# XinMing0411/zero-shot-AAC

Hardware: AMD Instinct MI355X
Metric: audio clips/sec end-to-end (encode+mapper+GPT-2 decode), Clotho-eval bs=64 (higher is better)
Workload: dtype bf16

## Files before the change

### zero-shot-aac_amd/csrc/decode_grid.hip

```cpp
#include <type_traits>

#include "common.h"

#pragma clang fp contract(off)

namespace zs {
int g_dp_spin = 0;
int g_dg_exp = 0;
int g_dg_dynf = 1;
int g_dp_abort = -1;
int g_dg_win_lo = 0;
int g_dg_win_hi = 62;
namespace dg {

constexpr int D = 768, NH = 12, HD = 64, DFF = 3072, NLY = 12, RM = 64, QKVN = 3 * D;
constexpr int NW = 4, NT = 64 * NW;
constexpr int KSD = D / 32, KSF = DFF / 32;
constexpr int QS = KSD / NW, QF = KSF / NW;
constexpr int NCB_Q = QKVN / 16, NCB_D = D / 16, NCB_F = DFF / 16;
constexpr unsigned SPIN_MAX = 1u << 22;
#ifndef DG_NSH
#define DG_NSH 8
#endif
constexpr int NSH = DG_NSH;
// ... 262 lines not shown
typedef __attribute__((ext_vector_type(2))) float f32x2_t;
__device__ __forceinline__ float dot2bf(unsigned x, unsigned y, float c) {
  return __builtin_amdgcn_fdot2_f32_bf16(__builtin_bit_cast(bf16x2_t, x), __builtin_bit_cast(bf16x2_t, y),
                                         c, false);
}
template <int NRB>
__device__ __forceinline__ void ln_stats(const u32x4_t* xf, const Sm& sm, int rb0) {
  const int tid = otid(), v = tid >> 6, lane = tid & 63, fr = lane & 15;
  constexpr unsigned ONE2 = 0x3f803f80u;
#pragma unroll
  for (int rb = 0; rb < NRB; ++rb) {
    float s = 0.f, q = 0.f;
#pragma unroll
    for (int i = 0; i < QS; ++i) {
      const u32x4_t u = xf[rb * QS + i];
      s = dot2bf(u.x, ONE2, s); q = dot2bf(u.x, u.x, q);
      s = dot2bf(u.y, ONE2, s); q = dot2bf(u.y, u.y, q);
      s = dot2bf(u.z, ONE2, s); q = dot2bf(u.z, u.z, q);
      s = dot2bf(u.w, ONE2, s); q = dot2bf(u.w, u.w, q);
    }
    s = add32(add16(s));
    q = add32(add16(q));
    if (lane < 16) {
      sm.ln[v * RM + 16 * (rb0 + rb) + fr] = s;
      sm.ln[(NW + v) * RM + 16 * (rb0 + rb) + fr] = q;
    }
  }
}
__device__ __forceinline__ void ln_row(const Sm& sm, int r, float& mean, float& rstd) {
  const float* l2 = sm.ln + NW * RM;
  mean = ((sm.ln[r] + sm.ln[RM + r]) + (sm.ln[2 * RM + r] + sm.ln[3 * RM + r])) * (1.0f / D);
  const float ex2 = ((l2[r] + l2[RM + r]) + (l2[2 * RM + r] + l2[3 * RM + r])) * (1.0f / D);
  rstd = rsqrtf(fmaxf(fmaf(-mean, mean, ex2), 0.f) + 1e-5f);
}
template <int NC>
__device__ __forceinline__ void stage_cb(const Sm& sm, const float* b2, int N, int n0) {
  static_assert(NC <= 64, "SM_CB holds 64 columns");
  const int t = otid();
  if (t < NC) sm.cb[t] = b2[n0 + t];
  else if (t >= 64 && t < 64 + NC) sm.cb[t] = b2[N + n0 + t - 64];
}
__device__ __forceinline__ float4 cb_quad(const Sm& sm, int lc, int row1) {
  return *reinterpret_cast<const float4*>(sm.cb + 64 * row1 + lc);
}
__device__ __forceinline__ float4 ln_fold(f32x4_t s, float mean, float rstd, float4 cs, float4 b) {
  return make_float4(fmaf(rstd, fmaf(-mean, cs.x, s[0]), b.x), fmaf(rstd, fmaf(-mean, cs.y, s[1]), b.y),
                     fmaf(rstd, fmaf(-mean, cs.z, s[2]), b.z), fmaf(rstd, fmaf(-mean, cs.w, s[3]), b.w));
}

template <int NRB>
__device__ __forceinline__ void embed_frags(const Args& a, const Sm& sm, int rb0, u32x4_t* xf) {
  const int tid = otid(), v = tid >> 6, lane = tid & 63, fr = lane & 15, fk = 8 * (lane >> 4);
#pragma unroll
  for (int rb = 0; rb < NRB; ++rb) {
    const int row = 16 * (rb0 + rb) + fr;
    const bf16_t* te = a.wte + (long)sm.tok[row] * D + fk;
#pragma unroll
    for (int i = 0; i < QS; ++i)
      xf[rb * QS + i] = *reinterpret_cast<const u32x4_t*>(te + 32 * (QS * v + i));
  }
#pragma unroll
  for (int rb = 0; rb < NRB; ++rb) {
    const int row = 16 * (rb0 + rb) + fr;
    const bf16_t* pe = a.wpe + (long)sm.pos[row] * D + fk;
    u32x4_t pu[QS];
#pragma unroll
    for (int i = 0; i < QS; ++i) pu[i] = *reinterpret_cast<const u32x4_t*>(pe + 32 * (QS * v + i));
#pragma unroll
    for (int i = 0; i < QS; ++i) {
      float t[8], p[8];
      unpack8(xf[rb * QS + i], t);
      unpack8(pu[i], p);
#pragma unroll
      for (int e = 0; e < 8; ++e) t[e] += p[e];
      xf[rb * QS + i] = pack8(t);
    }
  }
}
__device__ __forceinline__ float4 embed_quad(const Args& a, const Sm& sm, int row, int col) {
  const uint2 t = *reinterpret_cast<const uint2*>(a.wte + (long)sm.tok[row] * D + col);
  const uint2 p = *reinterpret_cast<const uint2*>(a.wpe + (long)sm.pos[row] * D + col);
  return make_float4(__uint_as_float(t.x << 16) + __uint_as_float(p.x << 16),
                     __uint_as_float(t.x & 0xffff0000u) + __uint_as_float(p.x & 0xffff0000u),
                     __uint_as_float(t.y << 16) + __uint_as_float(p.y << 16),
                     __uint_as_float(t.y & 0xffff0000u) + __uint_as_float(p.y & 0xffff0000u));
}

template <int CB, int RB>
struct Rounds {
  static constexpr int CPR = CB < 8 / RB ? CB : 8 / RB;
  static constexpr int NR = (CB + CPR - 1) / CPR;
  static constexpr int NJ = (CPR * RB + NW - 1) / NW;
};
template <int CB, int RB, int PF, typename LoadW, typename Epi>
__device__ __forceinline__ void gemm_rounds(const u32x4_t* xf, u32x4_t* wpf, f32x4_t* red,
                                            LoadW&& loadw, Epi&& epi) {
  constexpr int CPR = Rounds<CB, RB>::CPR, NR = Rounds<CB, RB>::NR;
  static_assert(PF == CB || PF == CPR, "weight prefetch rounds");
  static_for<NR>([&](auto rr) {
    constexpr int r = decltype(rr)::value, c0 = r * CPR;
    constexpr int NC = CB - c0 < CPR ? CB - c0 : CPR;
    f32x4_t acc[NC * RB];
#pragma unroll
    for (int t = 0; t < NC * RB; ++t) acc[t] = f32x4_t{0.f, 0.f, 0.f, 0.f};
#pragma unroll
    for (int s = 0; s < QS; ++s)
#pragma unroll
      for (int c = 0; c < NC; ++c)
#pragma unroll
        for (int rb = 0; rb < RB; ++rb)
          acc[c * RB + rb] = mfma(wpf[((PF == CB ? c0 : 0) + c) * QS + s], xf[rb * QS + s], acc[c * RB + rb]);
    if constexpr (PF != CB && c0 + CPR < CB) {
      loadw(c0 + CPR, std::integral_constant<int, (CB - c0 - CPR < CPR ? CB - c0 - CPR : CPR)>{}, wpf);
      __builtin_amdgcn_sched_barrier(0);
    }
    reduce_tiles<NC * RB>(red, acc, [&](int j, int t, f32x4_t s) { epi(r, j, c0 + t / RB, t % RB, s); });
  });
}

template <int G, bool PM>
__device__ __forceinline__ void phase_a(const Args& a, const Rs& rs, int l, int w, const Sm& sm,
                                        u32x4_t* wq) {
  using Gm = Geo<G>;
  constexpr int CB = Gm::ACB, RB = Gm::ARB, NCG = NCB_Q / CB;
  const int tid = otid(), v = tid >> 6, lane = tid & 63;
  const int cb0 = (w % NCG) * CB, rb0 = (w / NCG) * RB;
  u32x4_t xf[RB * QS];
  if (l == 0) embed_frags<RB>(a, sm, rb0, xf);
  else lda<RB, QS>(rs.xb, KSD, rb0, QS * v, xf);
  if constexpr (PM) ldw<Gm::APF, QS>(a.wq[l], KSD, cb0, QS * v, wq);
  stage_cb<16 * CB>(sm, a.bq[l], QKVN, 16 * cb0);
  __builtin_amdgcn_sched_barrier(0);
  ln_stats<RB>(xf, sm, rb0);
  const __amdgpu_buffer_rsrc_t rk = mk(a.kc[l], a.kv_bytes), rv = mk(a.vc[l], a.kv_bytes);
  gemm_rounds<CB, RB, Gm::APF>(xf, wq, sm.red,
      [&](int c, auto n, u32x4_t* wr) { ldw<decltype(n)::value, QS>(a.wq[l], KSD, cb0 + c, QS * (otid() >> 6), wr); },
      [&](int r, int j, int c, int rb, f32x4_t s) {
        const int row = 16 * (rb0 + rb) + (lane & 15), col = 16 * (cb0 + c) + 4 * (lane >> 4);
        if (row >= a.R) return;
        float mean, rstd;
        ln_row(sm, row, mean, rstd);
        const int lc = 16 * c + 4 * (lane >> 4);
        const float4 o4 = ln_fold(s, mean, rstd, cb_quad(sm, lc, 1), cb_quad(sm, lc, 0));
        const u32x2_t o{pk2bf(o4.x, o4.y), pk2bf(o4.z, o4.w)};
        if (col < D) {
          st8(rs.q, (row * D + col) * 2, o);
        } else {
          const int j = col - D, kv = j >= D, jj = kv ? j - D : j;
          const int off = ((((row * NH + jj / HD) * a.Lmax) + sm.pos[row]) * HD + (jj % HD)) * 2;
          st8(kv ? rv : rk, off, o);
        }
      });
}

__device__ __forceinline__ float gelu_new_fast(float x) {
  const float u2 = -1.5957691216057308f * fmaf(0.044715f * x * x, x, x);
  return x * __builtin_amdgcn_rcpf(1.0f + __expf(u2));
}
template <int G, bool PM>
__device__ __forceinline__ void phase_d(const Args& a, const Rs& rs, int l, int w, const Sm& sm,
                                        u32x4_t* wf) {
  using Gm = Geo<G>;
  constexpr int CB = Gm::DCB, RB = Gm::DRB, NCG = NCB_F / CB;
  const int tid = otid(), v = tid >> 6, lane = tid & 63;
  const int cb0 = (w % NCG) * CB, rb0 = (w / NCG) * RB;
  u32x4_t xf[RB * QS];
  lda<RB, QS>(rs.xb, KSD, rb0, QS * v, xf);
  if constexpr (PM) ldw<Gm::DPF, QS>(a.wf[l], KSD, cb0, QS * v, wf);
  stage_cb<16 * CB>(sm, a.bfc[l], DFF, 16 * cb0);
  __builtin_amdgcn_sched_barrier(0);
  ln_stats<RB>(xf, sm, rb0);
  gemm_rounds<CB, RB, Gm::DPF>(xf, wf, sm.red,
      [&](int c, auto n, u32x4_t* wr) { ldw<decltype(n)::value, QS>(a.wf[l], KSD, cb0 + c, QS * (otid() >> 6), wr); },
      [&](int r, int j, int c, int rb, f32x4_t s) {
        const int row = 16 * (rb0 + rb) + (lane & 15), col = 16 * (cb0 + c) + 4 * (lane >> 4);
        if (row >= a.R) return;
        float mean, rstd;
        ln_row(sm, row, mean, rstd);
        const int lc = 16 * c + 4 * (lane >> 4);
        const float4 h = ln_fold(s, mean, rstd, cb_quad(sm, lc, 1), cb_quad(sm, lc, 0));
        st8(rs.hid, frag_off(row, col, KSF),
            u32x2_t{pk2bf(gelu_new_fast(h.x), gelu_new_fast(h.y)),
                    pk2bf(gelu_new_fast(h.z), gelu_new_fast(h.w))});
      });
}

template <int G>
__device__ __forceinline__ void ce_tile(int w, int t, int& row, int& col) {
  using Gm = Geo<G>;
  constexpr int NCG = NCB_D / Gm::ECB;
  const int lane = otid() & 63;
  const int cb0 = (w % NCG) * Gm::ECB, rb0 = (w / NCG) * Gm::ERB;
  row = 16 * (rb0 + t % Gm::ERB) + (lane & 15);
  col = 16 * (cb0 + t / Gm::ERB) + 4 * (lane >> 4);
}
template <int G, bool PM>
__device__ __forceinline__ void ce_operands(const Args& a, const Sm& sm, bool embed, int w,
                                            const float* bias, const f32x4_t& xo, float4& b,
                                            float4& xold) {
  constexpr int T = Geo<G>::ECB * Geo<G>::ERB;
  const int v = otid() >> 6;
  b = make_float4(0.f, 0.f, 0.f, 0.f);
  xold = b;
  if (v < T) {
    int row, col;
    ce_tile<G>(w, v, row, col);
    b = *reinterpret_cast<const float4*>(bias + col);
    if (embed) {
      xold = embed_quad(a, sm, row, col);
    } else if constexpr (PM) {
      xold = *reinterpret_cast<const float4*>(reinterpret_cast<const float*>(a.ws + WS_X) + row * D + col);
    } else {
      xold = make_float4(xo[0], xo[1], xo[2], xo[3]);
    }
  }
}
template <int G, bool PM>
__device__ __forceinline__ void ce_epilogue(const Args& a, const Rs& rs, int w, int t, f32x4_t s,
                                            const float4& b, const float4& xold, f32x4_t& xo) {
  int row, col;
  ce_tile<G>(w, t, row, col);
  const f32x4_t o{(s[0] + b.x) + xold.x, (s[1] + b.y) + xold.y, (s[2] + b.z) + xold.z,
                  (s[3] + b.w) + xold.w};
  xo = o;
  if (row < a.R) {
    st8(rs.xb, frag_off(row, col, KSD), u32x2_t{pk2bf(o[0], o[1]), pk2bf(o[2], o[3])});
    if constexpr (PM)
      *reinterpret_cast<float4*>(reinterpret_cast<float*>(a.ws + WS_X) + row * D + col) =
          make_float4(o[0], o[1], o[2], o[3]);
  }
}

template <int G, bool PM>
__device__ __forceinline__ void phase_c(const Args& a, const Rs& rs, int l, int w, const Sm& sm,
                                        u32x4_t* wo, f32x4_t& xo) {
  using Gm = Geo<G>;
  constexpr int CB = Gm::ECB, RB = Gm::ERB, T = CB * RB, NCG = NCB_D / CB;
  const int v = otid() >> 6;
  const int cb0 = (w % NCG) * CB, rb0 = (w / NCG) * RB;
  u32x4_t af[RB * QS];
  lda<RB, QS>(rs.att, KSD, rb0, QS * v, af);
  if constexpr (PM) ldw<CB, QS>(a.wo[l], KSD, cb0, QS * v, wo);
  float4 b, xold;
  ce_operands<G, PM>(a, sm, l == 0, w, a.bo[l], xo, b, xold);
  __builtin_amdgcn_sched_barrier(0);
  f32x4_t acc[T];
#pragma unroll
  for (int t = 0; t < T; ++t) acc[t] = f32x4_t{0.f, 0.f, 0.f, 0.f};
#pragma unroll
  for (int s = 0; s < QS; ++s)
#pragma unroll
    for (int c = 0; c < CB; ++c)
#pragma unroll
      for (int rb = 0; rb < RB; ++rb) acc[c * RB + rb] = mfma(wo[c * QS + s], af[rb * QS + s], acc[c * RB + rb]);
  reduce_tiles<T>(sm.red, acc, [&](int, int t, f32x4_t s) { ce_epilogue<G, PM>(a, rs, w, t, s, b, xold, xo); });
}

template <int G, bool PM>
__device__ __forceinline__ void phase_e(const Args& a, const Rs& rs, int l, int w, const Sm& sm,
                                        u32x4_t* wm, f32x4_t& xo) {
  using Gm = Geo<G>;
  constexpr int CB = Gm::ECB, RB = Gm::ERB, T = CB * RB, NCG = NCB_D / CB, NCH = QF / ECH, ESL = Gm::ESL;
  const int v = otid() >> 6;
  const int cb0 = (w % NCG) * CB, rb0 = (w / NCG) * RB, s0 = QF * v;
  if constexpr (PM) {
#pragma unroll
    for (int k = 0; k < ESL; ++k) ldw<CB, ECH>(a.wm[l], KSF, cb0, s0 + ECH * k, wm + k * CB * ECH);
  }
  u32x4_t af[ESL * RB * ECH];
#pragma unroll
  for (int k = 0; k < ESL; ++k) lda<RB, ECH>(rs.hid, KSF, rb0, s0 + ECH * k, af + k * RB * ECH);
  float4 b, xold;
  ce_operands<G, PM>(a, sm, false, w, a.bm[l], xo, b, xold);
  __builtin_amdgcn_sched_barrier(0);
  f32x4_t acc[T];
#pragma unroll
  for (int t = 0; t < T; ++t) acc[t] = f32x4_t{0.f, 0.f, 0.f, 0.f};
  static_for<NCH>([&](auto cc) {
    constexpr int c = decltype(cc)::value, sl = c % ESL;
#pragma unroll
    for (int s = 0; s < ECH; ++s)
#pragma unroll
      for (int cb = 0; cb < CB; ++cb)
#pragma unroll
        for (int rb = 0; rb < RB; ++rb)
          acc[cb * RB + rb] = mfma(wm[(sl * CB + cb) * ECH + s], af[(sl * RB + rb) * ECH + s], acc[cb * RB + rb]);
    if constexpr (c + ESL < NCH) {
      ldw<CB, ECH>(a.wm[l], KSF, cb0, s0 + ECH * (c + ESL), wm + sl * CB * ECH);
      lda<RB, ECH>(rs.hid, KSF, rb0, s0 + ECH * (c + ESL), af + sl * RB * ECH);
      __builtin_amdgcn_sched_barrier(0);
    }
  });
  reduce_tiles<T>(sm.red, acc, [&](int, int t, f32x4_t s) { ce_epilogue<G, PM>(a, rs, w, t, s, b, xold, xo); });
}

__device__ __forceinline__ void attn_unit(const Args& a, const Sm& sm, int u, int& row, int& hh,
                                          int& p, long& base) {
  row = u / NH;
  hh = u % NH;
  const int rr = min(row, a.R - 1);
  p = (a.exp & 2) ? 1 : min(sm.pos[rr], a.Lmax - 1);
  base = ((long)(rr * NH + hh) * a.Lmax) * HD + 8 * ((otid() & 63) & 7);
}
template <int KU, int KC>
__device__ __forceinline__ void attn_load(const Args& a, int l, const Sm& sm, int ub, int cb,
                                          u32x4_t (&kr)[KU][KC], u32x4_t (&vr)[KU][KC]) {
  const int tid = otid(), v = tid >> 6, grp = (tid & 63) >> 3;
  const bf16_t* kc = a.kc[l];
  const bf16_t* vc = a.vc[l];
#pragma unroll
  for (int k = 0; k < KU; ++k) {
    int row, hh, p;
    long base;
    attn_unit(a, sm, ub + KU * v + k, row, hh, p, base);
#pragma unroll
    for (int i = 0; i < KC; ++i) {
      const int jc = max(min(cb + 8 * i + grp, p - 1), 0);
      kr[k][i] = __builtin_nontemporal_load(reinterpret_cast<const u32x4_t*>(kc + base + (long)jc * HD));
      vr[k][i] = __builtin_nontemporal_load(reinterpret_cast<const u32x4_t*>(vc + base + (long)jc * HD));
    }
  }
}
template <int KU, int KC>
__device__ __forceinline__ void phase_b(const Args& a, const Rs& rs, int l, const Sm& sm, int ub,
                                        u32x4_t (&kr)[KU][KC], u32x4_t (&vr)[KU][KC]) {
  const int tid = otid(), lane = tid & 63, v = tid >> 6, grp = lane >> 3, sub = lane & 7;
  const __amdgpu_buffer_rsrc_t rk = mk(a.kc[l], a.kv_bytes), rv = mk(a.vc[l], a.kv_bytes);
  float m[KU], sum[KU];
  f32x2_t o[KU][4];
  int p[KU], row[KU], hh[KU];
  long base[KU];
  u32x4_t qu[KU], knu[KU], vnu[KU];
#pragma unroll
  for (int k = 0; k < KU; ++k) {
    attn_unit(a, sm, ub + KU * v + k, row[k], hh[k], p[k], base[k]);
    qu[k] = ld16(rs.q, (min(row[k], a.R - 1) * D + hh[k] * HD + 8 * sub) * 2);
    const int off = (int)((base[k] + (long)p[k] * HD) * 2);
    knu[k] = ld16(rk, off);
    vnu[k] = ld16(rv, off);
  }
  __builtin_amdgcn_sched_barrier(0);
  auto qk = [&](const u32x4_t& qv, const u32x4_t& kv) {
    float sv = dot2bf(qv.x, kv.x, 0.f);
    sv = dot2bf(qv.y, kv.y, sv);
    sv = dot2bf(qv.z, kv.z, sv);
    sv = dot2bf(qv.w, kv.w, sv);
    return sum8(sv) * 0.125f;
  };
#pragma unroll
  for (int k = 0; k < KU; ++k) {
    m[k] = qk(qu[k], knu[k]);
    sum[k] = grp == 0 ? 1.f : 0.f;
    const unsigned w[4] = {vnu[k].x, vnu[k].y, vnu[k].z, vnu[k].w};
#pragma unroll
    for (int t = 0; t < 4; ++t)
      o[k][t] = grp == 0 ? f32x2_t{__uint_as_float(w[t] << 16), __uint_as_float(w[t] & 0xffff0000u)}
                         : f32x2_t{0.f, 0.f};
  }
  auto vacc = [&](f32x2_t (&acc)[4], float e, const u32x4_t& vv) {
    const unsigned w[4] = {vv.x, vv.y, vv.z, vv.w};
    const f32x2_t e2 = {e, e};
#pragma unroll
    for (int t = 0; t < 4; ++t)
      acc[t] = __builtin_elementwise_fma(e2, f32x2_t{__uint_as_float(w[t] << 16),
                                                     __uint_as_float(w[t] & 0xffff0000u)}, acc[t]);
  };
  int pmax = p[0];
#pragma unroll
  for (int k = 1; k < KU; ++k) pmax = max(pmax, p[k]);
  for (int cb = 0; cb < pmax; cb += 8 * KC) {
    if (cb > 0) attn_load<KU, KC>(a, l, sm, ub, cb, kr, vr);
#pragma unroll
    for (int h = 0; h < KC / 4; ++h) {
      const int cs = cb + 32 * h;
#pragma unroll
      for (int k = 0; k < KU; ++k) {
        if (cs >= p[k]) continue;
        float sc[4];
        float pm = -INFINITY;
#pragma unroll
        for (int i = 0; i < 4; ++i) {
          const float sv = qk(qu[k], kr[k][4 * h + i]);
          sc[i] = cs + 8 * i + grp < p[k] ? sv : -INFINITY;
          pm = fmaxf(pm, sc[i]);
        }
        pm = fmaxf(pm, xor8(pm));
        pm = max16(pm);
        pm = max32(pm);
        const float mn = fmaxf(m[k], pm);
        const float scale = __expf(m[k] - mn);
        sum[k] *= scale;
        const f32x2_t sc2 = {scale, scale};
#pragma unroll
        for (int t = 0; t < 4; ++t) o[k][t] *= sc2;
        m[k] = mn;
#pragma unroll
        for (int i = 0; i < 4; ++i) {
          const float e = __expf(sc[i] - mn);
          sum[k] += e;
          vacc(o[k], e, vr[k][4 * h + i]);
        }
      }
    }
  }
#pragma unroll
  for (int k = 0; k < KU; ++k) {
    const float inv = 1.0f / add32(add16(sum[k] + xor8(sum[k])));
    float of[8];
#pragma unroll
    for (int t = 0; t < 4; ++t) {
      of[2 * t] = add32(add16(o[k][t].x + xor8(o[k][t].x))) * inv;
      of[2 * t + 1] = add32(add16(o[k][t].y + xor8(o[k][t].y))) * inv;
    }
    if (grp == 0 && row[k] < a.R) {
      const int r = row[k];
      st16(rs.att, (((r >> 4) * KSD + 2 * hh[k] + (sub >> 2)) * 64 + (r & 15) + 16 * (sub & 3)) * 16,
           pack8(of));
    }
  }
}

template <int G, bool DYN>
__device__ __forceinline__ void phase_f(const Args& a, const Rs& rs, int w, const Sm& sm, gu64* keys,
                                        gu32* fctr) {
  const int tid = otid(), v = tid >> 6, lane = tid & 63;
  u32x4_t xf[4 * QS];
  lda<4, QS>(rs.xb, KSD, 0, QS * v, xf);
  const int nvb = (a.V + 15) >> 4, lmv = 16 * nvb;
  constexpr int NSL = Geo<G>::FSL;
  int su = (nvb + G * NSL - 1) / (G * NSL);
  bool dyn = false;
  if constexpr (DYN) {
    const int s2 = max(3, (nvb * 5 / 8) / (G * NSL));
    if (G * NSL * s2 <= nvb - G && a.exp == 0 && a.dynf) { su = s2; dyn = true; }
  }
  const int d0 = G * NSL * su, nch = dyn ? (nvb - d0 + NSL - 1) / NSL : 0;
  int* const chr = sm.misc + 12;
  auto iter_blocks = [&](int u, int& b0, int& st) {
    if (u < su) { b0 = w + G * NSL * u; st = G; }
    else if (dyn) { b0 = d0 + NSL * __builtin_amdgcn_readfirstlane(chr[u & 3]); st = 1; }
    else { b0 = 0x3fffffff; st = 0; }
  };
  static_assert(Geo<G>::FSL % 2 == 0 && Geo<G>::FSL >= 2, "F ring: an even number of slots");
  struct Slot {
    u32x4_t w[QS];
  };
  Slot R[NSL];
  auto fill = [&](int b, Slot& r) { ldw<1, QS>(a.wtep, KSD, min(max(b, 0), nvb - 1), QS * v, r.w); };
  float4 bq[2], cq[2];
  auto fill_b = [&](int b, float4& bb, float4& c) {
    const int bc = min(max(b, 0), nvb - 1);
    bb = *reinterpret_cast<const float4*>(a.lmb + 16 * bc + 4 * (lane >> 4));
    c = *reinterpret_cast<const float4*>(a.lmb + lmv + 16 * bc + 4 * (lane >> 4));
  };
  static_for<NSL>([&](auto k) { fill(w + G * decltype(k)::value, R[decltype(k)::value]); });
  fill_b(w, bq[0], cq[0]);
  __builtin_amdgcn_sched_barrier(0);
  ln_stats<4>(xf, sm, 0);
  float bv = -INFINITY;
  int bi = 0x7fffffff;
  const bool tmp = a.temp != 1.0f;
  int buf = 0;
  lds_sync();
  float mean, rstd;
  ln_row(sm, 16 * v + (lane & 15), mean, rstd);
  auto consume = [&](int b, const Slot& r, const float4& rb_, const float4& rc_) {
    f32x4_t acc[4];
#pragma unroll
    for (int rb = 0; rb < 4; ++rb) acc[rb] = f32x4_t{0.f, 0.f, 0.f, 0.f};
#pragma unroll
    for (int s = 0; s < QS; ++s)
#pragma unroll
      for (int rb = 0; rb < 4; ++rb) acc[rb] = mfma(r.w[s], xf[rb * QS + s], acc[rb]);
    f32x4_t* red = sm.red + buf * 1024;
#pragma unroll
    for (int rb = 0; rb < 4; ++rb) red[(v * 4 + rb) * 64 + lane] = acc[rb];
    lds_sync();
    const f32x4_t sum = (red[v * 64 + lane] + red[(4 + v) * 64 + lane]) +
                        (red[(8 + v) * 64 + lane] + red[(12 + v) * 64 + lane]);
    const int col0 = 16 * b + 4 * (lane >> 4);
    const float4 lg4 = ln_fold(sum, mean, rstd, rc_, rb_);
    const float lgv[4] = {lg4.x, lg4.y, lg4.z, lg4.w};
#pragma unroll
    for (int e = 0; e < 4; ++e) {
      const float lg = lgv[e];
      const float val = tmp ? lg / a.temp : lg;
      if (col0 + e < a.V && val > bv) { bv = val; bi = col0 + e; }
    }
    buf ^= 1;
  };
  unsigned pend = 0;
  int bu, stu;
  iter_blocks(0, bu, stu);
#pragma nounroll
  for (int u = 0; bu < nvb && u < su + nch; ++u) {
    int bn, stn;
    iter_blocks(u + 1, bn, stn);
    static_for<NSL>([&](auto kk) {
      constexpr int k = decltype(kk)::value;
      const int b = bu + k * stu;
      if (b < nvb) {
        fill_b(k + 1 < NSL ? b + stu : bn, bq[(k + 1) % 2], cq[(k + 1) % 2]);
        consume(b, R[k], bq[k % 2], cq[k % 2]);
      }
      if constexpr (k == 1) {
        if (dyn && tid == 0 && u >= su - 3) {
          if (u >= su - 2) chr[(u + 2) & 3] = (int)pend;
          pend = __hip_atomic_fetch_add(fctr, 1u, __ATOMIC_RELAXED, __HIP_MEMORY_SCOPE_AGENT);
        }
      }
      fill(bn + k * stn, R[k]);
    });
    bu = bn;
    stu = stn;
  }
#pragma unroll
  for (int o = 16; o < 64; o <<= 1) {
    const float ov = __shfl_xor(bv, o, 64);
    const int oi = __shfl_xor(bi, o, 64);
    if (ov > bv || (ov == bv && oi < bi)) { bv = ov; bi = oi; }
  }
  if (lane < 16) {
    const unsigned long long key = ((unsigned long long)f2key(bv) << 32) | (unsigned)(~bi);
    __hip_atomic_fetch_max(keys + 16 * v + lane, key, __ATOMIC_RELAXED, __HIP_MEMORY_SCOPE_AGENT);
  }
}

template <typename A>
__device__ __forceinline__ void load_state(const A& a, const Sm& sm) {
  const int tid = otid();
  if (tid < RM) {
    const bool in = tid < a.R;
    sm.tok[tid] = in ? a.next_tok[tid] : 0;
    sm.pos[tid] = in ? a.pos[tid] : 0;
    sm.done[tid] = in ? a.done[tid] : 1;
  }
}
template <typename A>
__device__ __forceinline__ void bookkeep(const A& a, const Sm& sm, gu64* keys, int step, bool commit) {
  const int tid = otid();
  int alive = 0;
  if (tid < RM) {
    const unsigned long long key = __hip_atomic_load(keys + tid, __ATOMIC_RELAXED, __HIP_MEMORY_SCOPE_AGENT);
    const int t = min(max((int)~(unsigned)key, 0), a.V - 1);
    if (tid < a.R) {
      int d = sm.done[tid];
      if (!d) {
        if (commit) {
          a.out_ids[(long)tid * a.max_steps + step] = t;
          a.out_len[tid] = step + 1;
        }
        if (t == a.stop0 || t == a.stop1) d = 1;
      }
      alive = !d;
      sm.done[tid] = d;
      sm.tok[tid] = t;
      sm.pos[tid] += 1;
      if (commit) {
        a.done[tid] = d;
        a.pos[tid] = sm.pos[tid];
        a.next_tok[tid] = t;
      }
    }
  }
  const unsigned long long bal = __ballot(alive);
  if (tid == 0) sm.misc[0] = (int)__popcll(bal);
}

template <typename A>
__device__ __forceinline__ void gave_up(const A& a) {
  if (threadIdx.x == 0) {
    __hip_atomic_store(&a.all_done[1], -1, __ATOMIC_RELAXED, __HIP_MEMORY_SCOPE_AGENT);
    __hip_atomic_store(&a.all_done[0], 1, __ATOMIC_RELAXED, __HIP_MEMORY_SCOPE_AGENT);
  }
}

template <int G>
__global__ __launch_bounds__(NT, 2) void dg_persist_kernel(Args a) {
  using Gm = Geo<G>;
  constexpr int KU = Units<G>::KU, KC = Units<G>::KC;
  __shared__ __attribute__((aligned(16))) char smem[SM_TOTAL];
  const Sm sm(smem);
  const int w = blockIdx.x;
  if (a.all_done[0]) return;
  int step = *a.step_ctr;
  if (step >= a.max_steps) return;
  load_state(a, sm);
  __syncthreads();
  const Rs rs = make_rs(a.ws, a.exp);
  Bar bar{(gu32*)(a.ws + WS_SH), (gu32*)(a.ws + WS_TMO), 0, G / NSH, a.spin_max, nullptr, 0};
  gu64* const keys = (gu64*)(a.ws + WS_KEY);
  gu32* const clm = (gu32*)(a.ws + WS_CLM);
  volatile lds_int_t* s_ok = (volatile lds_int_t*)(sm.misc + 8);
  unsigned long long* const stamps =
      (dp_stamp_ws == nullptr || dp_stamp_ws == a.ws) ? dp_stamp_buf : nullptr;
  const int stamp_step = dp_stamp_step;
  if (stamp_step == -2 && threadIdx.x == 0) {
    unsigned hw, xcc;
    asm volatile("s_getreg_b32 %0, hwreg(HW_REG_HW_ID)" : "=s"(hw));
    asm volatile("s_getreg_b32 %0, hwreg(HW_REG_XCC_ID)" : "=s"(xcc));
    ((gu64*)(a.ws + WS_X))[w] = ((unsigned long long)xcc << 32) | hw;
  }
  const int ub = w * Units<G>::UPG;
  constexpr int ANCG = NCB_Q / Gm::ACB, DNCG = NCB_F / Gm::DCB, ENCG = NCB_D / Gm::ECB;
  const int acb0 = (w % ANCG) * Gm::ACB, dcb0 = (w % DNCG) * Gm::DCB, ecb0 = (w % ENCG) * Gm::ECB;
#define V_ (otid() >> 6)
  u32x4_t wq[Gm::APF * QS];
  ldw<Gm::APF, QS>(a.wq[0], KSD, acb0, QS * V_, wq);
  f32x4_t xo{0.f, 0.f, 0.f, 0.f};
  for (;;) {
    bar.sb = (stamps != nullptr && step == stamp_step) ? stamps + (long)w * 2 * DP_NB : nullptr;
    bar.n0 = bar.n;
    stamp(bar.sb, 2 * DP_NB - 1);
    if (step == a.abort_step) return gave_up(a);
    for (int l = 0; l < NLY; ++l) {
      phase_a<G, false>(a, rs, l, w, sm, wq);
      bar_arrive(bar, w);
      u32x4_t kr[KU][KC], vr[KU][KC];
      attn_load<KU, KC>(a, l, sm, ub, 0, kr, vr);
      if (!bar_wait(bar, s_ok)) return gave_up(a);
      if (l == 0 && w == 0 && otid() < RM) {
        __hip_atomic_store(keys + ((step + 1) & 1) * RM + otid(), 0ull, __ATOMIC_RELAXED,
                           __HIP_MEMORY_SCOPE_AGENT);
        if (otid() == 0)
          __hip_atomic_store(clm + (CLM_F + ((step + 1) & 1)) * 32, 0u, __ATOMIC_RELAXED,
                             __HIP_MEMORY_SCOPE_AGENT);
      }
      phase_b<KU, KC>(a, rs, l, sm, ub, kr, vr);
      bar_arrive(bar, w);
      u32x4_t wo[Gm::ECB * QS];
      ldw<Gm::ECB, QS>(a.wo[l], KSD, ecb0, QS * V_, wo);
      if (!bar_wait(bar, s_ok)) return gave_up(a);
      phase_c<G, false>(a, rs, l, w, sm, wo, xo);
      bar_arrive(bar, w);
      u32x4_t wf[Gm::DPF * QS];
      ldw<Gm::DPF, QS>(a.wf[l], KSD, dcb0, QS * V_, wf);
      if (!bar_wait(bar, s_ok)) return gave_up(a);
      phase_d<G, false>(a, rs, l, w, sm, wf);
      bar_arrive(bar, w);
      u32x4_t wm[Gm::ESL * Gm::ECB * ECH];
#pragma unroll
      for (int k = 0; k < Gm::ESL; ++k)
        ldw<Gm::ECB, ECH>(a.wm[l], KSF, ecb0, QF * V_ + ECH * k, wm + k * Gm::ECB * ECH);
      if (!bar_wait(bar, s_ok)) return gave_up(a);
      phase_e<G, false>(a, rs, l, w, sm, wm, xo);
      bar_arrive(bar, w);
      if (l + 1 < NLY) ldw<Gm::APF, QS>(a.wq[l + 1], KSD, acb0, QS * V_, wq);
      else for (int i = 0; i < Gm::APF * QS; ++i) wq[i] = u32x4_t{0u, 0u, 0u, 0u};
      if (!bar_wait(bar, s_ok)) return gave_up(a);
    }
    phase_f<G, true>(a, rs, w, sm, keys + (step & 1) * RM, clm + (CLM_F + (step & 1)) * 32);
    bar_arrive(bar, w);
    ldw<Gm::APF, QS>(a.wq[0], KSD, acb0, QS * V_, wq);
    if (!bar_wait(bar, s_ok)) return gave_up(a);
    bookkeep(a, sm, keys + (step & 1) * RM, step, w == 0);
    __syncthreads();
    stamp(bar.sb, 2 * DP_NB - 2);
    const int total = sm.misc[0];
    const bool fin = total == 0 || step + 1 >= a.max_steps;
    if (w == 0 && otid() == 0) {
      *a.step_ctr = step + 1;
      a.all_done[2] = total;
      if (fin) a.all_done[0] = 1;
    }
    if (fin) return;
    ++step;
    __syncthreads();
  }
#undef V_
}

enum { PH_A = 0, PH_B, PH_C, PH_D, PH_E, PH_F };
template <int G, int PH>
__global__ __launch_bounds__(NT, 2) void dg_phase_kernel(Args a) {
  using Gm = Geo<G>;
  __shared__ __attribute__((aligned(16))) char smem[SM_TOTAL];
  const Sm sm(smem);
  const int w = blockIdx.x, l = a.layer;
  if (a.all_done[0]) return;
  if (*a.step_ctr >= a.max_steps) return;
  load_state(a, sm);
  __syncthreads();
  const Rs rs = make_rs(a.ws, a.exp);
  if constexpr (PH == PH_A) {
    u32x4_t wq[Gm::APF * QS];
    phase_a<G, true>(a, rs, l, w, sm, wq);
  } else if constexpr (PH == PH_B) {
    constexpr int KU = Units<G>::KU, KC = Units<G>::KC;
    u32x4_t kr[KU][KC], vr[KU][KC];
    attn_load<KU, KC>(a, l, sm, w * Units<G>::UPG, 0, kr, vr);
    phase_b<KU, KC>(a, rs, l, sm, w * Units<G>::UPG, kr, vr);
  } else if constexpr (PH == PH_C) {
    u32x4_t wo[Gm::ECB * QS];
    f32x4_t xo{0.f, 0.f, 0.f, 0.f};
    phase_c<G, true>(a, rs, l, w, sm, wo, xo);
  } else if constexpr (PH == PH_D) {
    u32x4_t wf[Gm::DPF * QS];
    phase_d<G, true>(a, rs, l, w, sm, wf);
  } else if constexpr (PH == PH_E) {
    u32x4_t wm[Gm::ESL * Gm::ECB * ECH];
    f32x4_t xo{0.f, 0.f, 0.f, 0.f};
    phase_e<G, true>(a, rs, l, w, sm, wm, xo);
  } else {
    phase_f<G, false>(a, rs, w, sm, (gu64*)(a.ws + WS_KEY), nullptr);
  }
}
template <typename A>
__global__ __launch_bounds__(64) void dg_book_kernel(A a) {
  __shared__ __attribute__((aligned(16))) char smem[SM_TOTAL];
  const Sm sm(smem);
  if (a.all_done[0]) return;
  const int step = *a.step_ctr;
  if (step >= a.max_steps) return;
  load_state(a, sm);
  __syncthreads();
  gu64* keys = (gu64*)(a.ws + WS_KEY);
  bookkeep(a, sm, keys, step, true);
  __syncthreads();
  if (threadIdx.x < RM) keys[threadIdx.x] = 0ull;
  if (threadIdx.x == 0) {
    const int total = sm.misc[0];
    *a.step_ctr = step + 1;
    a.all_done[2] = total;
    if (total == 0 || step + 1 >= a.max_steps) a.all_done[0] = 1;
  }
}

namespace f32 {
constexpr int KSD = D / 16, KSF = DFF / 16;
constexpr int QS = KSD / NW, QF = KSF / NW;
constexpr int G = 192;
constexpr int ACB = 3, ARB = 1, DCB = 2, DRB = 2, ECB = 1, ERB = 1;
constexpr int APF = 3;
constexpr int UPG = RM * NH / G, KC = 8;
constexpr int ESL = 4;
constexpr int FH = G / 2;

constexpr int WS_Q = WS_SYNC_BYTES;
constexpr int WS_ATT = WS_Q + RM * D * 4;
constexpr int WS_XB = WS_ATT + RM * D * 4;
constexpr int WS_HID = WS_XB + RM * D * 4;
constexpr int WS_BYTES = WS_HID + RM * DFF * 4;
constexpr int SM_TOTAL32 = SM_TOTAL;

struct Args {
  int R, Lmax, max_steps, stop0, stop1, V, layer, abort_step;
  unsigned spin_max;
  int kv_bytes;
  float temp;
  const float* wte; const float* wpe;
  const float* wq[NLY]; const float* bq[NLY];
  const float* wo[NLY]; const float* bo[NLY];
  const float* wf[NLY]; const float* bfc[NLY];
  const float* wm[NLY]; const float* bm[NLY];
  const float* wtep;
  const float* lmb;
  float* kc[NLY]; float* vc[NLY];
  int* pos; int* next_tok; int* done; int* out_ids; int* out_len; int* step_ctr; int* all_done;
  char* ws;
};

struct Rs {
  __amdgpu_buffer_rsrc_t q, att, xb, hid;
};
__device__ __forceinline__ Rs make_rs(char* ws) {
  return Rs{mk(ws + WS_Q, RM * D * 4), mk(ws + WS_ATT, RM * D * 4), mk(ws + WS_XB, RM * D * 4),
            mk(ws + WS_HID, RM * DFF * 4)};
}

__device__ __forceinline__ f32x4_t mfma4(const u32x4_t& w, const u32x4_t& a, f32x4_t c) {
  c = __builtin_amdgcn_mfma_f32_16x16x4f32(__uint_as_float(w.x), __uint_as_float(a.x), c, 0, 0, 0);
  c = __builtin_amdgcn_mfma_f32_16x16x4f32(__uint_as_float(w.y), __uint_as_float(a.y), c, 0, 0, 0);
  c = __builtin_amdgcn_mfma_f32_16x16x4f32(__uint_as_float(w.z), __uint_as_float(a.z), c, 0, 0, 0);
  return __builtin_amdgcn_mfma_f32_16x16x4f32(__uint_as_float(w.w), __uint_as_float(a.w), c, 0, 0, 0);
}
template <int NB, int S>
__device__ __forceinline__ void ldw(const float* Wp, int KS, int cb0, int s0, u32x4_t* w) {
  const __amdgpu_buffer_rsrc_t r = mk(const_cast<float*>(Wp), 0x7ffffff0);
  const int vo = ((cb0 * KS + s0) * 64 + (otid() & 63)) * 16;
#pragma unroll
  for (int nb = 0; nb < NB; ++nb)
#pragma unroll
    for (int s = 0; s < S; ++s) w[nb * S + s] = __builtin_amdgcn_raw_buffer_load_b128(r, vo, (nb * KS + s) * 1024, 0);
}
template <int NRB, int S>
__device__ __forceinline__ void lda(__amdgpu_buffer_rsrc_t r, int KS, int rb0, int s0, u32x4_t* a) {
  const int vo = ((rb0 * KS + s0) * 64 + (otid() & 63)) * 16;
#pragma unroll
  for (int rb = 0; rb < NRB; ++rb)
#pragma unroll
    for (int s = 0; s < S; ++s) a[rb * S + s] = __builtin_amdgcn_raw_buffer_load_b128(r, vo, (rb * KS + s) * 1024, 16);
}
__device__ __forceinline__ int frag_off(int row, int col, int KS) {
  return (((row >> 4) * KS + (col >> 4)) * 64 + (row & 15) + 16 * ((col >> 2) & 3)) * 16;
}
__device__ __forceinline__ u32x4_t u4(const float4& f) {
  return u32x4_t{__float_as_uint(f.x), __float_as_uint(f.y), __float_as_uint(f.z), __float_as_uint(f.w)};
}
__device__ __forceinline__ float4 f4(const u32x4_t& u) {
  return make_float4(__uint_as_float(u.x), __uint_as_float(u.y), __uint_as_float(u.z), __uint_as_float(u.w));
}
__device__ __forceinline__ float4 add4(const float4& a, const float4& b) {
  return make_float4(a.x + b.x, a.y + b.y, a.z + b.z, a.w + b.w);
}

template <int NRB>
__device__ __forceinline__ void ln_apply(u32x4_t* xf, const Sm& sm, int rb0) {
  const int tid = otid(), v = tid >> 6, lane = tid & 63, fr = lane & 15;
#pragma unroll
  for (int rb = 0; rb < NRB; ++rb) {
    float s = 0.f;
#pragma unroll
    for (int i = 0; i < QS; ++i) {
      const float4 x = f4(xf[rb * QS + i]);
      s += (x.x + x.y) + (x.z + x.w);
    }
    s = add32(add16(s));
    if (lane < 16) sm.ln[v * RM + 16 * (rb0 + rb) + fr] = s;
  }
  lds_sync();
#pragma unroll
  for (int rb = 0; rb < NRB; ++rb) {
    const int r = 16 * (rb0 + rb) + fr;
    const float mean = ((sm.ln[r] + sm.ln[RM + r]) + (sm.ln[2 * RM + r] + sm.ln[3 * RM + r])) * (1.0f / D);
    float q = 0.f;
#pragma unroll
    for (int i = 0; i < QS; ++i) {
      const float4 x = f4(xf[rb * QS + i]);
      const float4 d = make_float4(x.x - mean, x.y - mean, x.z - mean, x.w - mean);
      q += (d.x * d.x + d.y * d.y) + (d.z * d.z + d.w * d.w);
      xf[rb * QS + i] = u4(d);
    }
    q = add32(add16(q));
    if (lane < 16) sm.ln[(NW + v) * RM + r] = q;
  }
  lds_sync();
#pragma unroll
  for (int rb = 0; rb < NRB; ++rb) {
    const int r = 16 * (rb0 + rb) + fr;
    const float* l2 = sm.ln + NW * RM;
    const float var = ((l2[r] + l2[RM + r]) + (l2[2 * RM + r] + l2[3 * RM + r])) * (1.0f / D);
    const float rstd = rsqrtf(var + 1e-5f);
#pragma unroll
    for (int i = 0; i < QS; ++i) {
      const float4 d = f4(xf[rb * QS + i]);
      xf[rb * QS + i] = u4(make_float4(d.x * rstd, d.y * rstd, d.z * rstd, d.w * rstd));
    }
  }
}

template <int NRB>
__device__ __forceinline__ void embed_frags(const Args& a, const Sm& sm, int rb0, u32x4_t* xf) {
  const int tid = otid(), v = tid >> 6, lane = tid & 63, fr = lane & 15, fk = 4 * (lane >> 4);
#pragma unroll
  for (int rb = 0; rb < NRB; ++rb) {
    const int row = 16 * (rb0 + rb) + fr;
    const float* te = a.wte + (long)sm.tok[row] * D + fk;
    const float* pe = a.wpe + (long)sm.pos[row] * D + fk;
#pragma unroll
    for (int i = 0; i < QS; ++i)
      xf[rb * QS + i] = u4(add4(*reinterpret_cast<const float4*>(te + 16 * (QS * v + i)),
                                *reinterpret_cast<const float4*>(pe + 16 * (QS * v + i))));
  }
}
__device__ __forceinline__ float4 embed_quad(const Args& a, const Sm& sm, int row, int col) {
  return add4(*reinterpret_cast<const float4*>(a.wte + (long)sm.tok[row] * D + col),
              *reinterpret_cast<const float4*>(a.wpe + (long)sm.pos[row] * D + col));
}

template <int CB, int RB, typename Epi>
__device__ __forceinline__ void gemm_tiles(const u32x4_t* xf, const u32x4_t* wr, const Sm& sm, Epi&& epi) {
  f32x4_t acc[CB * RB];
#pragma unroll
  for (int t = 0; t < CB * RB; ++t) acc[t] = f32x4_t{0.f, 0.f, 0.f, 0.f};
#pragma unroll
  for (int s = 0; s < QS; ++s)
#pragma unroll
    for (int c = 0; c < CB; ++c)
#pragma unroll
      for (int rb = 0; rb < RB; ++rb) acc[c * RB + rb] = mfma4(wr[c * QS + s], xf[rb * QS + s], acc[c * RB + rb]);
  reduce_tiles<CB * RB>(sm.red, acc, epi);
}
template <int CB, int RB>
__device__ __forceinline__ float4 bias_quad(const float* b, int cb0) {
  const int tid = otid(), v = tid >> 6, lane = tid & 63;
  if (v >= CB * RB) return make_float4(0.f, 0.f, 0.f, 0.f);
  return *reinterpret_cast<const float4*>(b + 16 * (cb0 + v / RB) + 4 * (lane >> 4));
}

template <bool PM>
__device__ __forceinline__ void phase_a(const Args& a, const Rs& rs, int l, int w, const Sm& sm, u32x4_t* wq) {
  constexpr int CB = ACB, RB = ARB, NCG = NCB_Q / CB;
  const int tid = otid(), v = tid >> 6, lane = tid & 63;
  const int cb0 = (w % NCG) * CB, rb0 = (w / NCG) * RB;
  u32x4_t xf[RB * QS];
  if (l == 0) embed_frags<RB>(a, sm, rb0, xf);
  else lda<RB, QS>(rs.xb, KSD, rb0, QS * v, xf);
  if constexpr (PM) ldw<APF, QS>(a.wq[l], KSD, cb0, QS * v, wq);
  u32x4_t wr[CB * QS];
#pragma unroll
  for (int i = 0; i < APF * QS; ++i) wr[i] = wq[i];
  ldw<CB - APF, QS>(a.wq[l], KSD, cb0 + APF, QS * v, wr + APF * QS);
  const float4 bq = bias_quad<CB, RB>(a.bq[l], cb0);
  __builtin_amdgcn_sched_barrier(0);
  ln_apply<RB>(xf, sm, rb0);
  const __amdgpu_buffer_rsrc_t rk = mk(a.kc[l], a.kv_bytes), rv = mk(a.vc[l], a.kv_bytes);
  gemm_tiles<CB, RB>(xf, wr, sm, [&](int, int t, f32x4_t s) {
    const int row = 16 * (rb0 + t % RB) + (lane & 15), col = 16 * (cb0 + t / RB) + 4 * (lane >> 4);
    if (row >= a.R) return;
    const u32x4_t o = u4(make_float4(s[0] + bq.x, s[1] + bq.y, s[2] + bq.z, s[3] + bq.w));
    if (col < D) {
      st16(rs.q, (row * D + col) * 4, o);
    } else {
      const int j = col - D, kv = j >= D, jj = kv ? j - D : j;
      st16(kv ? rv : rk, ((((row * NH + jj / HD) * a.Lmax) + sm.pos[row]) * HD + (jj % HD)) * 4, o);
    }
  });
}

template <bool PM>
__device__ __forceinline__ void phase_d(const Args& a, const Rs& rs, int l, int w, const Sm& sm, u32x4_t* wf) {
  constexpr int CB = DCB, RB = DRB, NCG = NCB_F / CB;
  const int tid = otid(), v = tid >> 6, lane = tid & 63;
  const int cb0 = (w % NCG) * CB, rb0 = (w / NCG) * RB;
  u32x4_t xf[RB * QS];
  lda<RB, QS>(rs.xb, KSD, rb0, QS * v, xf);
  if constexpr (PM) ldw<CB, QS>(a.wf[l], KSD, cb0, QS * v, wf);
  const float4 bq = bias_quad<CB, RB>(a.bfc[l], cb0);
  __builtin_amdgcn_sched_barrier(0);
  ln_apply<RB>(xf, sm, rb0);
  gemm_tiles<CB, RB>(xf, wf, sm, [&](int, int t, f32x4_t s) {
    const int row = 16 * (rb0 + t % RB) + (lane & 15), col = 16 * (cb0 + t / RB) + 4 * (lane >> 4);
    if (row >= a.R) return;
    st16(rs.hid, frag_off(row, col, KSF),
         u4(make_float4(act_apply(s[0] + bq.x, ACT_GELU_TANH), act_apply(s[1] + bq.y, ACT_GELU_TANH),
                        act_apply(s[2] + bq.z, ACT_GELU_TANH), act_apply(s[3] + bq.w, ACT_GELU_TANH))));
  });
}

__device__ __forceinline__ void ce_tile(int w, int& row, int& col) {
  constexpr int NCG = NCB_D / ECB;
  const int lane = otid() & 63;
  row = 16 * ((w / NCG) * ERB) + (lane & 15);
  col = 16 * ((w % NCG) * ECB) + 4 * (lane >> 4);
}
template <bool PM>
__device__ __forceinline__ void ce_operands(const Args& a, const Rs& rs, const Sm& sm, bool embed, int w,
                                            const float* bias, const f32x4_t& xo, float4& b, float4& xold) {
  const int v = otid() >> 6;
  b = make_float4(0.f, 0.f, 0.f, 0.f);
  xold = b;
  if (v == 0) {
    int row, col;
// ... 631 lines not shown
```

Before: 7936.

## Software-pipeline attention KV loads by prefetching next chunk per slot

Restructures the decode attention loop so that K and V registers for the next chunk are loaded right after each slot's values are consumed, instead of loading the whole chunk at the top of each iteration. The final chunk is peeled into a separate instantiation without prefetch. Positions are made wave-uniform via readfirstlane, and row and head are recomputed at store time to save registers. This is meant to hide global-memory latency behind the softmax and accumulate math, at the cost of register pressure and code size. It also tightens a static_assert on the F ring size and zeroes xo before phase F.

```diff
diff --git a/zero-shot-aac_amd/csrc/decode_grid.hip b/zero-shot-aac_amd/csrc/decode_grid.hip
--- a/zero-shot-aac_amd/csrc/decode_grid.hip
+++ b/zero-shot-aac_amd/csrc/decode_grid.hip
@@ -588,6 +588,10 @@
   p = (a.exp & 2) ? 1 : min(sm.pos[rr], a.Lmax - 1);
   base = ((long)(rr * NH + hh) * a.Lmax) * HD + 8 * ((otid() & 63) & 7);
 }
+__device__ __forceinline__ u32x4_t attn_ld(const bf16_t* c, long base, int j, int p) {
+  const int jc = max(min(j, p - 1), 0);
+  return __builtin_nontemporal_load(reinterpret_cast<const u32x4_t*>(c + base + (long)jc * HD));
+}
 template <int KU, int KC>
 __device__ __forceinline__ void attn_load(const Args& a, int l, const Sm& sm, int ub, int cb,
                                           u32x4_t (&kr)[KU][KC], u32x4_t (&vr)[KU][KC]) {
@@ -601,9 +605,8 @@
     attn_unit(a, sm, ub + KU * v + k, row, hh, p, base);
 #pragma unroll
     for (int i = 0; i < KC; ++i) {
-      const int jc = max(min(cb + 8 * i + grp, p - 1), 0);
-      kr[k][i] = __builtin_nontemporal_load(reinterpret_cast<const u32x4_t*>(kc + base + (long)jc * HD));
-      vr[k][i] = __builtin_nontemporal_load(reinterpret_cast<const u32x4_t*>(vc + base + (long)jc * HD));
+      kr[k][i] = attn_ld(kc, base, cb + 8 * i + grp, p);
+      vr[k][i] = attn_ld(vc, base, cb + 8 * i + grp, p);
     }
   }
 }
@@ -612,16 +615,21 @@
                                         u32x4_t (&kr)[KU][KC], u32x4_t (&vr)[KU][KC]) {
   const int tid = otid(), lane = tid & 63, v = tid >> 6, grp = lane >> 3, sub = lane & 7;
   const __amdgpu_buffer_rsrc_t rk = mk(a.kc[l], a.kv_bytes), rv = mk(a.vc[l], a.kv_bytes);
+  const bf16_t* kc = a.kc[l];
+  const bf16_t* vc = a.vc[l];
   float m[KU], sum[KU];
   f32x2_t o[KU][4];
-  int p[KU], row[KU], hh[KU];
-  long base[KU];
+  int p[KU];
+  int base[KU];
   u32x4_t qu[KU], knu[KU], vnu[KU];
 #pragma unroll
   for (int k = 0; k < KU; ++k) {
-    attn_unit(a, sm, ub + KU * v + k, row[k], hh[k], p[k], base[k]);
-    qu[k] = ld16(rs.q, (min(row[k], a.R - 1) * D + hh[k] * HD + 8 * sub) * 2);
-    const int off = (int)((base[k] + (long)p[k] * HD) * 2);
+    int row, hh;
+    long b;
+    attn_unit(a, sm, ub + KU * v + k, row, hh, p[k], b);
+    base[k] = (int)b;
+    qu[k] = ld16(rs.q, (min(row, a.R - 1) * D + hh * HD + 8 * sub) * 2);
+    const int off = (int)((b + (long)p[k] * HD) * 2);
     knu[k] = ld16(rk, off);
     vnu[k] = ld16(rv, off);
   }
@@ -651,44 +659,62 @@
       acc[t] = __builtin_elementwise_fma(e2, f32x2_t{__uint_as_float(w[t] << 16),
                                                      __uint_as_float(w[t] & 0xffff0000u)}, acc[t]);
   };
-  int pmax = p[0];
-#pragma unroll
-  for (int k = 1; k < KU; ++k) pmax = max(pmax, p[k]);
-  for (int cb = 0; cb < pmax; cb += 8 * KC) {
-    if (cb > 0) attn_load<KU, KC>(a, l, sm, ub, cb, kr, vr);
+  int ps[KU], pmax = 0;
+#pragma unroll
+  for (int k = 0; k < KU; ++k) {
+    ps[k] = __builtin_amdgcn_readfirstlane(p[k]);
+    pmax = max(pmax, ps[k]);
+  }
+  auto step = [&](int cb, auto more_) {
+    constexpr bool MORE = decltype(more_)::value;
 #pragma unroll
     for (int h = 0; h < KC / 4; ++h) {
-      const int cs = cb + 32 * h;
+      const int cs = cb + 32 * h, cn = cs + 8 * KC;
 #pragma unroll
       for (int k = 0; k < KU; ++k) {
-        if (cs >= p[k]) continue;
-        float sc[4];
+        const bool on = cs < ps[k];
+        float sc[4] = {-INFINITY, -INFINITY, -INFINITY, -INFINITY};
         float pm = -INFINITY;
-#pragma unroll
-        for (int i = 0; i < 4; ++i) {
-          const float sv = qk(qu[k], kr[k][4 * h + i]);
-          sc[i] = cs + 8 * i + grp < p[k] ? sv : -INFINITY;
-          pm = fmaxf(pm, sc[i]);
+        if (on) {
+#pragma unroll
+          for (int i = 0; i < 4; ++i) {
+            const float sv = qk(qu[k], kr[k][4 * h + i]);
+            sc[i] = cs + 8 * i + grp < ps[k] ? sv : -INFINITY;
+            pm = fmaxf(pm, sc[i]);
+          }
         }
-        pm = fmaxf(pm, xor8(pm));
-        pm = max16(pm);
-        pm = max32(pm);
-        const float mn = fmaxf(m[k], pm);
-        const float scale = __expf(m[k] - mn);
-        sum[k] *= scale;
-        const f32x2_t sc2 = {scale, scale};
-#pragma unroll
-        for (int t = 0; t < 4; ++t) o[k][t] *= sc2;
-        m[k] = mn;
-#pragma unroll
-        for (int i = 0; i < 4; ++i) {
-          const float e = __expf(sc[i] - mn);
-          sum[k] += e;
-          vacc(o[k], e, vr[k][4 * h + i]);
+        if constexpr (MORE) {
+#pragma unroll
+          for (int i = 0; i < 4; ++i) kr[k][4 * h + i] = attn_ld(kc, base[k], cn + 8 * i + grp, ps[k]);
+        }
+        if (on) {
+          pm = fmaxf(pm, xor8(pm));
+          pm = max16(pm);
+          pm = max32(pm);
+          const float mn = fmaxf(m[k], pm);
+          const float scale = __expf(m[k] - mn);
+          sum[k] *= scale;
+          const f32x2_t sc2 = {scale, scale};
+#pragma unroll
+          for (int t = 0; t < 4; ++t) o[k][t] *= sc2;
+          m[k] = mn;
+#pragma unroll
+          for (int i = 0; i < 4; ++i) {
+            const float e = __expf(sc[i] - mn);
+            sum[k] += e;
+            vacc(o[k], e, vr[k][4 * h + i]);
+          }
+        }
+        if constexpr (MORE) {
+#pragma unroll
+          for (int i = 0; i < 4; ++i) vr[k][4 * h + i] = attn_ld(vc, base[k], cn + 8 * i + grp, ps[k]);
         }
       }
     }
-  }
+  };
+  int cb = 0;
+  for (; cb + 8 * KC < pmax; cb += 8 * KC) step(cb, std::true_type{});
+  if (cb < pmax) step(cb, std::false_type{});
 #pragma unroll
   for (int k = 0; k < KU; ++k) {
     const float inv = 1.0f / add32(add16(sum[k] + xor8(sum[k])));
@@ -698,9 +724,9 @@
       of[2 * t] = add32(add16(o[k][t].x + xor8(o[k][t].x))) * inv;
       of[2 * t + 1] = add32(add16(o[k][t].y + xor8(o[k][t].y))) * inv;
     }
-    if (grp == 0 && row[k] < a.R) {
-      const int r = row[k];
-      st16(rs.att, (((r >> 4) * KSD + 2 * hh[k] + (sub >> 2)) * 64 + (r & 15) + 16 * (sub & 3)) * 16,
+    const int u = ub + KU * (otid() >> 6) + k, r = u / NH, hh = u % NH;
+    if (grp == 0 && r < a.R) {
+      st16(rs.att, (((r >> 4) * KSD + 2 * hh + (sub >> 2)) * 64 + (r & 15) + 16 * (sub & 3)) * 16,
            pack8(of));
     }
   }
@@ -727,7 +753,9 @@
     else if (dyn) { b0 = d0 + NSL * __builtin_amdgcn_readfirstlane(chr[u & 3]); st = 1; }
     else { b0 = 0x3fffffff; st = 0; }
   };
-  static_assert(Geo<G>::FSL % 2 == 0 && Geo<G>::FSL >= 2, "F ring: an even number of slots");
+  static_assert(Geo<G>::FSL % 2 == 0 && Geo<G>::FSL >= 4,
+                "F ring: an even number of slots, and a workgroup barrier between a claim's "
+                "publication (slot 1) and its read (the next iteration)");
   struct Slot {
     u32x4_t w[QS];
   };
@@ -935,6 +963,7 @@
       else for (int i = 0; i < Gm::APF * QS; ++i) wq[i] = u32x4_t{0u, 0u, 0u, 0u};
       if (!bar_wait(bar, s_ok)) return gave_up(a);
     }
+    xo = f32x4_t{0.f, 0.f, 0.f, 0.f};
     phase_f<G, true>(a, rs, w, sm, keys + (step & 1) * RM, clm + (CLM_F + (step & 1)) * 32);
     bar_arrive(bar, w);
     ldw<Gm::APF, QS>(a.wq[0], KSD, acb0, QS * V_, wq);
```

Result: no change. 8001 (median of 6 runs) (+0.8%).
